# anonymous-author-918/deq-mpc-corl

Measured on AMD Instinct MI355X. Metric: QP solves/sec at (B,T=20,nx=13,nu=4), higher is better.
Workload: dtype f32

## Files before the change

### deq-mpc-corl_amd/_lib.py

```python
from __future__ import annotations

import ctypes as C
import os

_HERE = os.path.dirname(os.path.abspath(__file__))
LIB_PATH = os.environ.get("MI_ALQP_LIB") or os.path.join(_HERE, "csrc", "libmi_alqp.so")

ABI_VERSION = 17


class AlqpDims(C.Structure):
    _fields_ = [("B", C.c_int), ("T", C.c_int), ("nx", C.c_int), ("nu", C.c_int)]


class AlqpParams(C.Structure):
    _fields_ = [("al_iter", C.c_int), ("max_newton", C.c_int), ("n_ls", C.c_int),
                ("flags", C.c_int), ("rho_scale", C.c_double), ("variant", C.c_int),
                ("skip_flag", C.c_void_p), ("exit_tol", C.c_double), ("newton_counts", C.c_void_p),
                ("exit_scratch", C.c_void_p), ("quad_stagger", C.c_int)]


class AlqpTrace(C.Structure):
    _fields_ = [("g", C.c_void_p), ("d", C.c_void_p), ("phi", C.c_void_p),
                ("phi_prev", C.c_void_p), ("k", C.c_void_p), ("accept", C.c_void_p)]


class AlqpObstacles(C.Structure):
    _fields_ = [("pos", C.c_void_p), ("radius", C.c_double), ("nobs", C.c_int), ("state_estimator", C.c_int)]


class AlqpBwdDyn(C.Structure):
    _fields_ = [("lam", C.c_void_p), ("sb_lam", C.c_long), ("dF", C.c_void_p), ("dc", C.c_void_p), ("dx0", C.c_void_p)]


class AlqpIpmParams(C.Structure):
    _fields_ = [("flags", C.c_int), ("max_iter", C.c_int), ("iter0", C.c_int), ("kkt_eps", C.c_double),
                ("variant", C.c_int)]


class AlqpRigidParams(C.Structure):
    _fields_ = [("mass", C.c_double), ("J", C.c_double * 9), ("Jinv", C.c_double * 9), ("g", C.c_double * 3),
                ("motor_dist", C.c_double), ("kf", C.c_double), ("bf", C.c_double), ("km", C.c_double),
                ("act_scale", C.c_double), ("u_hover", C.c_double), ("pend_L", C.c_double), ("ss", C.c_double * 12),
                ("bf_force", C.c_double)]


IPM_VARIANTS = {"auto": 0, "generic_lds": 1, "generic_ws": 2, "resident": 3}


ALQP_IPM_INIT, ALQP_IPM_RESID, ALQP_IPM_STEP, ALQP_IPM_LOOP, ALQP_IPM_FINAL = 1, 2, 4, 8, 16
ALQP_INIT_MERIT = 1
ALQP_DUAL_UPDATE = 2
ALQP_SAVE_FACTOR = 4
ALQP_WS_PRIMED = 8
ALQP_EXIT_IN_KERNEL = 16
ALQP_E_COOP = -4
VARIANT_AUTO, VARIANT_TEAM, VARIANT_QUAD = 0, 1, 2

ERRORS = {-1: "bad argument", -2: "unsupported (nx, nu), or horizon / batch beyond what the requested kernel can hold or address",
          -3: "kernel launch failed", -4: "grid too large for a cooperative launch"}

_P = C.c_void_p
_ROWS = (_P, _P, C.c_int, C.c_long, C.c_long, C.c_long, C.c_long)
_SIGS = {
    "alqp_solve_nonlin": (C.c_int, [C.POINTER(AlqpDims), C.POINTER(AlqpParams), C.c_int, C.c_double, _P, _P, _P, _P, _P,
                                    C.c_long, C.c_long, _P, _P, _P, _P, _P, _P, _P, _P, C.c_size_t, _P]),
    "alqp_solve_nonlin_rows": (C.c_int, [C.POINTER(AlqpDims), C.POINTER(AlqpParams), C.c_int, C.c_double, _P, _P, _P, _P, _P,
                                         C.c_long, C.c_long, _P, _P, C.c_long, C.c_long, *_ROWS, _P, _P, _P, _P, _P, _P, _P,
                                         _P, C.POINTER(AlqpTrace), _P, C.c_size_t, _P]),
    "alqp_dyn_pendulum1l": (C.c_int, [C.c_long, _P, _P, C.c_double, _P, _P, _P, _P]),
    "alqp_dyn_cartpole1l": (C.c_int, [C.c_long, _P, _P, C.c_double, _P, _P, _P, _P]),
    "alqp_dyn_cartpole1l_v2": (C.c_int, [C.c_long, _P, _P, C.c_double, _P, _P, _P, _P]),
    "alqp_dyn_cartpole2l": (C.c_int, [C.c_long, _P, _P, C.c_double, _P, _P, _P, _P]),
    "alqp_dyn_rexquadrotor": (C.c_int, [C.c_long, C.POINTER(AlqpRigidParams), _P, _P, C.c_double, _P, _P, _P]),
    "alqp_dyn_flyingcartpole": (C.c_int, [C.c_long, C.POINTER(AlqpRigidParams), _P, _P, C.c_double, _P, _P, _P]),
    "alqp_solve_lin": (C.c_int, [C.POINTER(AlqpDims), C.POINTER(AlqpParams), _P, _P, _P, _P, _P, _P, _P,
                                 C.c_long, C.c_long, _P, _P, _P, _P, _P, _P, _P, _P,
                                 C.POINTER(AlqpTrace), _P, C.c_size_t, _P]),
    "alqp_solve_lin_shared": (C.c_int, [C.POINTER(AlqpDims), C.POINTER(AlqpParams), _P, _P, _P, _P,
                                        C.c_long, C.c_long, C.c_long, C.c_long, _P, _P, _P,
                                        C.c_long, C.c_long, _P, _P, _P, _P, _P, _P, _P, _P,
                                        C.POINTER(AlqpTrace), _P, C.c_size_t, _P]),
    "alqp_solve_lin_dense": (C.c_int, [C.POINTER(AlqpDims), C.POINTER(AlqpParams), _P, _P, _P, _P, _P, _P, _P,
                                       C.c_long, C.c_long, _P, _P, _P, _P, _P, _P, _P, _P,
                                       C.POINTER(AlqpTrace), _P]),
    "alqp_solve_lin_xbox": (C.c_int, [C.POINTER(AlqpDims), C.POINTER(AlqpParams), _P, _P, _P, _P, _P, _P, _P,
                                      C.c_long, C.c_long, _P, _P, C.c_long, C.c_long, _P, _P, _P, _P, _P, _P, _P, _P,
                                      C.POINTER(AlqpTrace), _P]),
    "alqp_solve_lin_poly": (C.c_int, [C.POINTER(AlqpDims), C.POINTER(AlqpParams), _P, _P, _P, _P, _P, _P, _P,
                                      C.c_long, C.c_long, _P, _P, C.c_int, C.c_long, C.c_long, C.c_long, C.c_long,
                                      _P, _P, _P, _P, _P, _P, _P, _P, C.POINTER(AlqpTrace), _P]),
    "alqp_solve_lin_gen": (C.c_int, [C.POINTER(AlqpDims), C.POINTER(AlqpParams), _P, _P, _P, _P, _P, _P, _P,
                                     C.c_long, C.c_long, _P, _P, _P, _P, _P, _P, _P, _P,
                                     C.POINTER(AlqpTrace), _P, C.c_size_t, _P,
                                     _P, _P, _P, C.c_long, C.c_long, _P, _P, C.c_int, C.c_long, C.c_long, C.c_long, C.c_long]),
    "alqp_newton_step": (C.c_int, [C.POINTER(AlqpDims), _P, _P, _P, _P, _P, _P, _P, _P, _P, _P,
                                   C.c_long, C.c_long, C.POINTER(AlqpObstacles), _P, C.c_size_t, _P, _P, _P, _P, _P]),
    "alqp_merit": (C.c_int, [C.POINTER(AlqpDims), C.c_int, _P, _P, _P, _P, _P, _P, _P, _P, _P,
                             C.c_long, C.c_long, C.POINTER(AlqpObstacles), _P, _P, _P]),
    "alqp_linesearch_pick": (C.c_int, [C.POINTER(AlqpDims), C.c_int, _P, _P, _P, _P, _P, _P, _P]),
    "alqp_dual_update": (C.c_int, [C.POINTER(AlqpDims), _P, _P, _P, _P, _P, C.c_long, C.c_long,
                                   C.POINTER(AlqpObstacles), _P, _P, C.c_double, _P]),
    "alqp_backward": (C.c_int, [C.POINTER(AlqpDims), _P, _P, C.c_size_t, _P, _P, _P, _P, _P, _P,
                                C.POINTER(AlqpBwdDyn), _P]),
    "alqp_merit_pick": (C.c_int, [C.POINTER(AlqpDims), C.c_int, _P, _P, _P, _P, _P, _P, _P, _P, _P,
                                  C.c_long, C.c_long, C.POINTER(AlqpObstacles), _P, _P, _P, _P, _P, _P, _P]),
    "alqp_newton_step_xbox": (C.c_int, [C.POINTER(AlqpDims), _P, _P, _P, _P, _P, _P, _P, _P, _P, _P,
                                        C.c_long, C.c_long, _P, _P, C.c_long, C.c_long, _P, _P, _P, _P, _P]),
# ... 75 lines not shown
```

### deq-mpc-corl_amd/csrc/alqp_quad.hip

```cpp
#if defined(ALQP_BWD_DYN_UNIT) || defined(ALQP_SHDYN_UNIT)
#undef ALQP_PHASE_TIMING
#endif
#include <hip/hip_runtime.h>

#include "alqp_quad.hpp"
#include "alqp_dims.hpp"
#include "alqp_launch.hpp"

#if defined(ALQP_QUAD_F32) == defined(ALQP_QUAD_F64)
#error "compile alqp_quad.hip with exactly one of -DALQP_QUAD_F32, -DALQP_QUAD_F64"
#endif

namespace alqp {

#ifndef ALQP_FUSE_LS
#define ALQP_FUSE_LS 1
#endif
#ifdef ALQP_PHASE_TIMING
__device__ unsigned long long g_phase_cycles[10];
#define QSTAMP(b) qd.stamp(b)
#else
#define QSTAMP(b)
#endif
#ifdef ALQP_SHDYN_UNIT
template <typename real, int NX, int NU, bool TRACE, class Dyn = NoDyn>
__global__ __launch_bounds__(64) __attribute__((amdgpu_waves_per_eu(1, 1))) void k_solve_lin_quad_shdyn(ShdynSolveArgs<real> a, TraceArgs<real> tr, real *ws) {
#else
template <typename real, int NX, int NU, bool TRACE, class Dyn = NoDyn>
__global__ __launch_bounds__(64) __attribute__((amdgpu_waves_per_eu(1, 1))) void k_solve_lin_quad(SolveArgs<real> a, TraceArgs<real> tr, real *ws) {
#endif
    using C = QCfg<real, NX, NU>;
    constexpr bool NL = Dyn::ID != 0;
#ifndef ALQP_FUSE_LS_F64
#define ALQP_FUSE_LS_F64 1
#endif
    constexpr bool FUSE_LS = ALQP_FUSE_LS && (sizeof(real) == 4 || ALQP_FUSE_LS_F64) && !NL;
    constexpr int N = C::N;
    if (a.skip && *a.skip != 0.0) return;
    const int lane = threadIdx.x, qi = lane >> 2;
    const int b_raw = blockIdx.x * 16 + qi;
    const bool active = b_raw < a.B;
    {
        int stag = a.stagger;
        const int mode = (a.flags >> 20) & 0xf;
        if ((a.flags >> 24) & 0xff) stag = (a.flags >> 24) & 0xff;
        if (stag > 0) {
            const unsigned hw = __builtin_amdgcn_s_getreg(4 | (0 << 6) | (31 << 11));
            int simd = (hw >> 4) & 3;
            if (mode == 1) simd = simd * 16 + ((hw >> 8) & 0xf);
            if (mode == 2) simd &= 1;
            if (mode == 3) simd = blockIdx.x & 1;
            if (mode == 4) simd = (simd & 1) ^ (blockIdx.x & 1);
            if (mode == 5) simd = (hw >> 8) & 3;
            for (int i = 0; i < simd * stag; ++i) __builtin_amdgcn_s_sleep(16);
        }
    }
#ifdef ALQP_ALIAS_ALL
    const int b = (active ? b_raw : a.B - 1) % ALQP_ALIAS_ALL;
#else
    const int b = active ? b_raw : a.B - 1;
#endif
    const int T = a.T, M = C::M(T);

    Quad<real, NX, NU> qd;
    __shared__ real w_lds[QCfg<real, NX, NU>::WLDS_WORDS];
    qd.wl = w_lds + threadIdx.x;
    qd.q = lane & 3;
    qd.T = T;
    qd.active = active;
    qd.gQd = a.Qd + (size_t)b * T * N;
    qd.gq = a.q + (size_t)b * T * N;
#ifdef ALQP_SHDYN_UNIT
    qd.gF = a.F + (size_t)b * a.sb_F;
    qd.gc = a.c + (size_t)b * a.sb_c;
    qd.mt_F = a.mt_F; qd.mt_c = a.mt_c;
#else
    qd.gF = a.F + (size_t)b * (T - 1) * NX * N;
    qd.gc = a.c + (size_t)b * (T - 1) * NX;
#endif
    qd.gx0 = a.x0 + (size_t)b * NX;
    qd.gulo = a.ulo + (size_t)b * a.sb_u;
    qd.guhi = a.uhi + (size_t)b * a.sb_u;
    qd.st_u = a.st_u;
    qd.gz = a.z + (size_t)b * T * N;
    qd.glam = a.lam + (size_t)b * M;
    qd.rec = ws + C::rec_base(b, T);
    qd.gFw = const_cast<real *>(qd.gF);
    qd.dyn_h = a.dyn_h;
    qd.rho = a.rho[b];
    qd.info = 0;
    real phi_prev = a.phi[b];
#ifdef ALQP_PHASE_TIMING
    for (int i = 0; i < 10; ++i) qd.tacc[i] = 0;
#endif
    QSTAMP(-1);
    if (!(a.flags & ALQP_WS_PRIMED)) {
        if constexpr (NL) qd.stage_in(false, false);
        else qd.stage_in(a.max_newton == 0 || a.al_iter == 0 || (a.flags & ALQP_EXIT_IN_KERNEL) ||
                         (!C::PHI0_FWD && (a.flags & ALQP_INIT_MERIT)));
    }
    const bool ref_exit = (a.flags & ALQP_EXIT_IN_KERNEL) != 0;
    int gphase = 0;

    int step_id = 0;
    bool pend = false;
    real alpha_pend = 0;
    int bad = 0;
    real rn2 = 0, phi_next = 0;
    for (int it = 0; it < a.al_iter; ++it) {
        bool phi_from_forward = false;
        if (a.flags & ALQP_INIT_MERIT) {
            if (it > 0) {
                phi_prev = phi_next;
            } else if (C::PHI0_FWD && a.max_newton > 0 && !ref_exit) {
                phi_from_forward = true;
            } else {
                if constexpr (NL) qd.template linearize<Dyn>(real(0), false);
                real p1[1];
                qd.template merit_candidates<1>(p1, true);
                phi_prev = p1[0];
            }
        }
        pend = false;
        double nrm_old = 0;
        int n_done = 0;
        if (ref_exit) {
            int bad0 = 0;
            const real r0 = it == 0 ? qd.rplus2(bad0) : rn2;
            nrm_old = sqrt(grid_sum_ordered(wave_sum_leaders(exit_term(r0, qor(qd.info)), active && qd.q == 0), a.exit_scratch, gphase));
        }
        for (int st = 0; st < a.max_newton; ++st, ++step_id) {
            real *tg = nullptr;
            if constexpr (TRACE) tg = (tr.g && active) ? tr.g + ((size_t)step_id * a.B + b) * T * N : nullptr;
            QSTAMP(9);
            if constexpr (NL) {
                qd.template linearize<Dyn>(alpha_pend, pend);
                pend = false;
            }
            qd.forward(tg, alpha_pend, pend, (phi_from_forward && st == 0) ? &phi_prev : nullptr);
            real ph[20];
            const bool store_s = !FUSE_LS || ref_exit || st + 1 == a.max_newton;
            qd.template backward<FUSE_LS>(ph, nullptr, store_s);
            QSTAMP(-1);
            if constexpr (TRACE) {
                if (tr.d && active) {
                    real *td = tr.d + ((size_t)step_id * a.B + b) * T * N;
                    for (int t = 0; t < T; ++t)
                        for (int j = qd.q; j < N; j += 4) td[t * N + j] = qd.recp(t)[C::wn(C::oY, j)];
                }
            }
            if constexpr (NL) qd.template merit_nonlin<Dyn>(ph);
            else if constexpr (!FUSE_LS) qd.template merit_candidates<20>(ph, false);
            QSTAMP(6);
            int kbest = 0;
            real best = ph[0];
#pragma unroll
            for (int k = 1; k < 20; ++k) {
                if (k < a.n_ls && !(best != best) && (ph[k] != ph[k] || ph[k] < best)) {
                    best = ph[k];
                    kbest = k;
                }
            }
            const bool acc = best < phi_prev;
            if constexpr (TRACE) {
                if (active && qd.q == 0) {
                    if (tr.phi)
#pragma unroll
                        for (int k = 0; k < 20; ++k)
                            if (k < a.n_ls) tr.phi[((size_t)step_id * a.n_ls + k) * a.B + b] = ph[k];
                    if (tr.phi_prev) tr.phi_prev[(size_t)step_id * a.B + b] = phi_prev;
                    if (tr.k) tr.k[(size_t)step_id * a.B + b] = kbest;
                    if (tr.accept) tr.accept[(size_t)step_id * a.B + b] = acc ? 1 : 0;
                }
            }
            const real alpha = acc ? real(1) / real(1 << kbest) : real(0);
            pend = true;
            alpha_pend = alpha;
            QSTAMP(7);
            phi_prev = best;
            if (ref_exit) {
                int bad1 = 0;
                real ph_unused = 0, r1 = 0;
                qd.template iter_end<Dyn>(alpha_pend, pend, false, (real)a.rho_scale, false, ph_unused, r1, bad1);
                pend = false;
                const double nw = sqrt(grid_sum_ordered(wave_sum_leaders(exit_term(r1, qor(qd.info)), active && qd.q == 0), a.exit_scratch, gphase));
                ++n_done;
                if (nw < a.exit_tol || fabs(nrm_old - nw) / nw < a.exit_tol) break;
                nrm_old = nw;
            }
        }
        if (ref_exit && a.newton_counts && blockIdx.x == 0 && lane == 0) a.newton_counts[it] = grid_barrier_timed_out(a.exit_scratch) ? -1 : n_done;
        bad = 0;
        qd.template iter_end<Dyn>(alpha_pend, pend, (a.flags & ALQP_DUAL_UPDATE) != 0, (real)a.rho_scale, it + 1 == a.al_iter,
                    phi_next, rn2, bad);
        pend = false;
// ... 231 lines not shown
```

### deq-mpc-corl_amd/csrc/alqp_quad.hpp

```cpp
#pragma once
#include <hip/hip_runtime.h>

#include <type_traits>

#include "alqp_team.hpp"
#include "alqp_dyn.hpp"

namespace alqp {

template <int Q>
__device__ inline float qb(float v) {
    return __builtin_bit_cast(float, __builtin_amdgcn_mov_dpp(__builtin_bit_cast(int, v), Q * 0x55, 0xF, 0xF, true));
}
template <int Q>
__device__ inline double qb(double v) {
    long long b = __builtin_bit_cast(long long, v);
    int lo = __builtin_amdgcn_mov_dpp((int)(b & 0xffffffffll), Q * 0x55, 0xF, 0xF, true);
    int hi = __builtin_amdgcn_mov_dpp((int)(b >> 32), Q * 0x55, 0xF, 0xF, true);
    return __builtin_bit_cast(double, ((long long)hi << 32) | (unsigned int)lo);
}
template <typename real>
__device__ inline real qbv(real v, int src) {
    switch (src & 3) {
        case 0: return qb<0>(v);
        case 1: return qb<1>(v);
        case 2: return qb<2>(v);
        default: return qb<3>(v);
    }
}
template <int CTRL>
__device__ inline float qperm(float v) {
    return __builtin_bit_cast(float, __builtin_amdgcn_mov_dpp(__builtin_bit_cast(int, v), CTRL, 0xF, 0xF, true));
}
template <int CTRL>
__device__ inline double qperm(double v) {
    long long b = __builtin_bit_cast(long long, v);
    int lo = __builtin_amdgcn_mov_dpp((int)(b & 0xffffffffll), CTRL, 0xF, 0xF, true);
    int hi = __builtin_amdgcn_mov_dpp((int)(b >> 32), CTRL, 0xF, 0xF, true);
    return __builtin_bit_cast(double, ((long long)hi << 32) | (unsigned int)lo);
}
template <typename real>
__device__ inline real qsum(real v) {
    v += qperm<0xB1>(v);
    v += qperm<0x4E>(v);
    return v;
}
__device__ inline int qor(int v) {
    v |= __builtin_amdgcn_mov_dpp(v, 0xB1, 0xF, 0xF, true);
    v |= __builtin_amdgcn_mov_dpp(v, 0x4E, 0xF, 0xF, true);
    return v;
}
template <typename real>
__device__ inline real sel4(real a0, real a1, real a2, real a3, int q) {
    real lo = (q & 1) ? a1 : a0, hi = (q & 1) ? a3 : a2;
    return (q & 2) ? hi : lo;
}

struct __attribute__((packed, aligned(4))) f4u { float x, y, z, w; };
struct __attribute__((packed, aligned(8))) d4u { double x, y, z, w; };
__device__ inline void gld4(const float *p, float &a, float &b, float &c, float &d) {
    f4u t = *reinterpret_cast<const f4u *>(p);
    a = t.x; b = t.y; c = t.z; d = t.w;
}
__device__ inline void gld4(const double *p, double &a, double &b, double &c, double &d) {
    d4u t = *reinterpret_cast<const d4u *>(p);
    a = t.x; b = t.y; c = t.z; d = t.w;
}
__device__ inline void gst4(float *p, float a, float b, float c, float d) {
    f4u t; t.x = a; t.y = b; t.z = c; t.w = d;
    *reinterpret_cast<f4u *>(p) = t;
}
__device__ inline void gst4(double *p, double a, double b, double c, double d) {
    d4u t; t.x = a; t.y = b; t.z = c; t.w = d;
    *reinterpret_cast<d4u *>(p) = t;
}
template <int LEN, typename real>
__device__ inline void gload(const real *p, real (&dst)[LEN]) {
#pragma unroll
    for (int c = 0; c + 4 <= LEN; c += 4) gld4(p + c, dst[c], dst[c + 1], dst[c + 2], dst[c + 3]);
#pragma unroll
    for (int c = (LEN / 4) * 4; c < LEN; ++c) dst[c] = p[c];
}

#ifndef ALQP_W_LDS
#define ALQP_W_LDS 1
#endif
#ifndef ALQP_EXP_NOQ
#define ALQP_EXP_NOQ 0
#endif
#ifndef ALQP_EXP_NORS
#define ALQP_EXP_NORS 0
#endif
#ifndef ALQP_EXP_NOL
#define ALQP_EXP_NOL 0
#endif
template <typename real, int SW, int N, bool IN_LDS>
struct WPanel {
    real a[SW][N];
    __device__ __forceinline__ real (&operator[](int s))[N] { return a[s]; }
    __device__ __forceinline__ const real (&operator[](int s) const)[N] { return a[s]; }
};
template <typename real, int N>
struct WRowLds {
    real *p;
    __device__ __forceinline__ real &operator[](int k) const { return p[k * 64]; }
};
template <typename real, int SW, int N>
struct WPanel<real, SW, N, true> {
    real *base;
    __device__ __forceinline__ WRowLds<real, N> operator[](int s) const { return WRowLds<real, N>{base + s * N * 64}; }
};
template <int LEN, typename real>
__device__ __forceinline__ void gload(const real *p, WRowLds<real, LEN> row) {
    real tmp[LEN];
    gload<LEN>(p, tmp);
#pragma unroll
    for (int k = 0; k < LEN; ++k) row[k] = tmp[k];
}

struct NoDyn {
    static constexpr int ID = 0;
};

struct Fld {
    int h, t;
};
template <int H, int T>
struct FldT {
    static constexpr int h = H, t = T;
    __host__ __device__ constexpr operator Fld() const { return {H, T}; }
};
template <typename real>
struct FRef {
    real *p;
    Fld f;
};
template <typename real, int H, int T>
__device__ __forceinline__ FRef<std::remove_const_t<real>> operator+(real *p, FldT<H, T>) {
    return {const_cast<std::remove_const_t<real> *>(p), Fld{H, T}};
}

template <typename real, int NX_, int NU_>
struct QCfg {
    static constexpr int NX = NX_, NU = NU_, N = NX_ + NU_;
    static constexpr int SH = (N + 3) / 4;
    static constexpr int SW = (NX + 3) / 4;
    static constexpr int SY = SH;
    static constexpr int HT = 2 * SH * (SH + 1);
    __host__ __device__ static constexpr int hidx(int s, int j) { return 2 * s * (s + 1) + j; }
    static constexpr int ST = 2 * SW * (SW + 1);
    static constexpr int BLK = 64 / (int)sizeof(real);
#ifndef ALQP_REC_IL_F32
#define ALQP_REC_IL_F32 2
#endif
    static constexpr int IL = sizeof(real) == 4 ? ALQP_REC_IL_F32 : 1;
    static_assert(IL == 1 || BLK == 16, "groups of 16 words are 64-byte blocks");
    __host__ __device__ static constexpr int w(int x) { return (x / 16) * (16 * IL) + x % 16; }
    static constexpr int NLAST = N - 4 * (SH - 1);
    __host__ __device__ static constexpr int lanes_of(int s) { return s == SH - 1 ? NLAST : 4; }
    __host__ __device__ static constexpr int lstride(int s) { return lanes_of(s) == 3 ? 16 : 4 * lanes_of(s); }
    __host__ __device__ static constexpr int lbase(int s) {
        int o = 0;
        for (int i = 0; i < s; ++i) o += (i + 1) * lstride(i);
        return o;
    }
    static constexpr int LW = lbase(SH);
    static constexpr bool PHI0_FWD = sizeof(real) == 4;
#ifndef ALQP_S_AFTER_F32
#define ALQP_S_AFTER_F32 0
#endif
    static constexpr bool S_AFTER = sizeof(real) == 8 || ALQP_S_AFTER_F32;
#ifndef ALQP_W_LDS_F32
#define ALQP_W_LDS_F32 0
#endif
    static constexpr bool W_LDS = ALQP_W_LDS && (sizeof(real) == 8 || ALQP_W_LDS_F32);
    static constexpr int WLDS_WORDS = W_LDS ? SW * N * 64 : 1;
    __host__ __device__ static constexpr int p4(int x) { return (x + 3) & ~3; }
    static constexpr int NF = 9;
    __host__ __device__ static constexpr int fslots(int i) { return (i <= 1 || i == 6 || i == 7) ? SY : (i == 5 ? 4 : SW); }
    static constexpr int oL = 2 * 16 * (SY / 4);
    __host__ __device__ static constexpr int tail_at(int i) {
        int g = (oL + LW + 15) & ~15, o = 0;
        for (int k = 0; k < NF; ++k) {
            const int r = fslots(k) % 4;
            if (r > 0 && o + r > 4) { g += 16; o = 0; }
            if (k == i) return g + o;
            o += r;
        }
        return o > 0 ? g + 16 : g;
    }
    __host__ __device__ static constexpr int head_at(int i) {
        if (i < 2) return i * 16 * (SY / 4);
        int o = tail_at(NF);
        for (int k = 2; k < i; ++k) o += 16 * (fslots(k) / 4);
        return o;
    }
    static constexpr FldT<head_at(0), tail_at(0)> oY{};
    static constexpr FldT<head_at(1), tail_at(1)> oZ{};
    static constexpr FldT<head_at(2), tail_at(2)> oR{};
    static constexpr FldT<head_at(3), tail_at(3)> oS{};
    static constexpr FldT<head_at(4), tail_at(4)> oLE{};
    static_assert(NU <= 4, "the u-slot layout holds one control per lane");
    static constexpr FldT<head_at(5), tail_at(5)> oUS{};
    static constexpr FldT<head_at(6), tail_at(6)> oQ{};
    static constexpr FldT<head_at(7), tail_at(7)> oq{};
    static constexpr FldT<head_at(8), tail_at(8)> oC{};
    static constexpr int RECW = (head_at(NF) + 31) & ~31;
    static_assert(IL == 1 || RECW % 16 == 0, "whole groups per record");
    template <int S>
    __host__ __device__ static constexpr int lp(int m, int q) {
        return m < 4 * (S / 4) ? 16 * (m / 4) + 4 * q + m % 4 : 16 * (S / 4) + q * (S % 4) + m - 4 * (S / 4);
    }
    template <int S>
    __host__ __device__ static constexpr int fw(Fld f, int p) {
        return p < 16 * (S / 4) ? w(f.h + p) : w(f.t + 4 * ((p - 16 * (S / 4)) / (S % 4)) + (p - 16 * (S / 4)) % (S % 4));
    }
    __host__ __device__ static constexpr int pn(int k) { return lp<SY>(k >> 2, k & 3); }
    __host__ __device__ static constexpr int px(int r) { return lp<SW>(r >> 2, r & 3); }
    __host__ __device__ static constexpr int wn(Fld f, int k) { return fw<SY>(f, pn(k)); }
    __host__ __device__ static constexpr int M(int T) { return T * NX + 2 * T * NU; }
    static constexpr int RSTR = RECW * IL;
    __host__ __device__ static constexpr size_t rec_base(int b, int T) { return (size_t)(b / IL) * T * RSTR + (size_t)(b % IL) * 16; }
    __host__ __device__ static constexpr size_t ws_words(int B, int T) { return (size_t)((B + IL - 1) / IL) * T * RSTR; }
    __host__ static bool ws_covers(int B, int T) {
        return rec_base(B - 1, T) + (size_t)(T - 1) * RSTR + w(RECW - 1) + 1 <= ws_words(B, T);
    }
};

template <typename real, int NX, int NU>
struct Quad {
    using C = QCfg<real, NX, NU>;
    static constexpr int N = C::N, SH = C::SH, SW = C::SW, SY = C::SY, HT = C::HT, ST = C::ST, RECW = C::RECW;

    int q, T;
    bool active;
    const real *gQd, *gq, *gF, *gc, *gx0, *gulo, *guhi;
    long st_u;
#ifdef ALQP_SHDYN_UNIT
    int mt_F, mt_c;
#endif
    real *gz, *glam, *rec;
    real rho;
    int info;
    real *wl;
    using WT = WPanel<real, SW, N, C::W_LDS>;
    __device__ __forceinline__ WT wpanel() const {
        if constexpr (C::W_LDS) return WT{wl};
        else return WT{};
    }
    real *gFw;
    real dyn_h;
    const real *gobs;
    int nobs;
    real obs_r2;
    bool no_init;

    __device__ __forceinline__ real uhi(int t, int j) const { return guhi[t * st_u + j]; }
    __device__ __forceinline__ real ulo(int t, int j) const { return gulo[t * st_u + j]; }
    __device__ __forceinline__ real *recp(int t) const { return rec + (size_t)t * C::RSTR; }
#ifdef ALQP_PHASE_TIMING
    unsigned long long tacc[10], tlast;
    __device__ __forceinline__ void stamp(int bucket) {
        unsigned long long now;
        __builtin_amdgcn_sched_barrier(0);
        asm volatile("s_waitcnt vmcnt(0)\n\ts_memtime %0\n\ts_waitcnt lgkmcnt(0)" : "=s"(now)::"memory");
        __builtin_amdgcn_sched_barrier(0);
        if (bucket >= 0) tacc[bucket] += now - tlast;
        tlast = now;
    }
#define ALQP_STAMP(b) stamp(b)
#else
#define ALQP_STAMP(b)
#endif

    template <int S, int L>
    __device__ __forceinline__ void ld_slots(FRef<real> f, real (&v)[L]) const {
        static_assert(L <= S, "slots of the field");
#pragma unroll
        for (int c = 0; 4 * c < L && c < S / 4; ++c) {
            const real *p = f.p + C::w(f.f.h + 16 * c) + 4 * q;
            if (4 * c + 3 < L) gld4(p, v[4 * c], v[4 * c + 1], v[4 * c + 2], v[4 * c + 3]);
            else
#pragma unroll
                for (int i = 0; 4 * c + i < L; ++i) v[4 * c + i] = p[i];
        }
        constexpr int H = 4 * (S / 4), R = S % 4;
        if constexpr (L > H) {
            const real *p = f.p + C::w(f.f.t) + 4 * q;
#pragma unroll
            for (int m = H; m < L; ++m) v[m] = p[m - H];
        }
    }
    template <int S, int L0>
    __device__ __forceinline__ void ld_slots_from(FRef<real> f, real (&v)[S]) const {
        static_assert(L0 >= 0 && L0 <= S, "slots of the field");
#pragma unroll
        for (int c = L0 / 4; c < S / 4; ++c) {
            const real *p = f.p + C::w(f.f.h + 16 * c) + 4 * q;
            if (4 * c >= L0) gld4(p, v[4 * c], v[4 * c + 1], v[4 * c + 2], v[4 * c + 3]);
            else {
                real w[4];
                gld4(p, w[0], w[1], w[2], w[3]);
#pragma unroll
                for (int i = 0; i < 4; ++i)
                    if (4 * c + i >= L0) v[4 * c + i] = w[i];
            }
        }
        constexpr int H = 4 * (S / 4);
// ... 285 lines not shown
        const real a0 = sel4(real(1), real(0.5), real(0.25), real(0.125), q);
        for (int t = 0; t < T; ++t) {
            const bool dyn = t < T - 1;
            const real *rp = recp(t), *rn = recp(dyn ? t + 1 : t);
            real zt[N], dt[N], Qt[N], qt[N], zn[NX], dn[NX], le[NX], lu[NU], ll[NU], bu[NU], bl[NU];
            ld_rep_n(rp + C::oZ, zt);
            ld_rep_n(rp + C::oY, dt);
            ld_rep_n(rp + C::oQ, Qt);
            ld_rep_n(rp + C::oq, qt);
            ld_repx_of_n(rn + C::oZ, zn);
            ld_repx_of_n(rn + C::oY, dn);
            ld_rep_x(rp + C::oLE, le);
            ld_rep_us(rp, lu, ll, bu, bl);
            real alpha = a0;
#pragma unroll
            for (int i = 0; i < 5; ++i) {
                real zc[N];
                real acc = 0;
#pragma unroll
                for (int j = 0; j < N; ++j) {
                    zc[j] = fma_(alpha, dt[j], zt[j]);
                    acc = fma_(fma_(real(0.5) * Qt[j], zc[j], qt[j]), zc[j], acc);
                }
#pragma unroll
                for (int ju = 0; ju < NU; ++ju) {
                    const real vu = zc[NX + ju] - bu[ju], vl = bl[ju] - zc[NX + ju];
                    const real cu = fmax_(vu, real(0)), cl = fmax_(vl, real(0));
                    acc += fma_(lu[ju], vu, ll[ju] * vl) + real(0.5) * rho * fma_(cu, cu, cl * cl);
                }
                if (dyn) {
                    real xn[NX];
                    dyn_value<Dyn, real>(zc, dyn_h, xn);
#pragma unroll
                    for (int r = 0; r < NX; ++r) {
                        const real rr = fma_(alpha, dn[r], zn[r]) - xn[r];
                        acc = fma_(fma_(real(0.5) * rho, rr, le[r]), rr, acc);
                    }
                }
                if (t == 0) {
#pragma unroll
                    for (int r = 0; r < NX; ++r) {
                        const real rr = zc[r] - x0v[r];
                        acc = fma_(fma_(real(0.5) * rho, rr, li[r]), rr, acc);
                    }
                }
                m[i] += acc;
                alpha *= real(0.0625);
            }
        }
#pragma unroll
        for (int k = 0; k < 20; ++k) phi[k] = qbv(m[k >> 2], k);
    }

    template <bool EXT = false>
    __device__ __forceinline__ void forward(real *g_out, real alpha, bool pending, real *phi0, const real *gxn = nullptr) {
        real mdist = 0;
        real S[ST], Sy[SW];
        real vpo[SW], Syo[SW];
        real zc[SW];
#pragma unroll
        for (int i = 0; i < ST; ++i) S[i] = 0;
#pragma unroll
        for (int s = 0; s < SW; ++s) Sy[s] = 0;
        {
            real z0[SW], xi[SW], li[SW], r0[SW];
            if constexpr (EXT) {
                ld_own_ext<NX>(gz, z0);
                ld_own_ext<NX>(glam + (T - 1) * NX, li);
            } else {
                ld_ownx_of_n(recp(0) + C::oZ, z0);
                ld_own_x(recp(T - 1) + C::oLE, li);
            }
            ld_own_ext<NX>(gx0, xi);
            if (pending) {
                real d0[SW];
                ld_ownx_of_n(recp(0) + C::oY, d0);
#pragma unroll
                for (int s = 0; s < SW; ++s) z0[s] = fma_(alpha, d0[s], z0[s]);
            }
#pragma unroll
            for (int s = 0; s < SW; ++s) {
                bool valid = 4 * s + 3 < NX || 4 * s + q < NX;
                if constexpr (EXT) valid = valid && !no_init;
                const real r = valid ? z0[s] - xi[s] : real(0);
                vpo[s] = valid ? fma_(rho, r, li[s]) : real(0);
                if constexpr (C::PHI0_FWD) mdist += valid ? fma_(fma_(real(0.5) * rho, r, li[s]), r, real(0)) : real(0);
                Syo[s] = 0;
                r0[s] = r;
                zc[s] = z0[s];
            }
            if (!EXT && active) st_own_x(recp(T - 1) + C::oR, r0);
        }
        for (int t = 0; t < T; ++t) {
            const bool dyn = t < T - 1;
            WT W = wpanel();
            real Y[N];
            real dio[SY];
            real v[SW];
            real zs[SY];
            real hob[3] = {0, 0, 0};
            real *rp = recp(t);
            {
                real zt[N];
                real Qo[SY], qo[SY];
                real cs[SW], zn[SW], lm[SW];
                real lu, ll, bu, bl;
                const int td = dyn ? t : (T > 1 ? T - 2 : 0);
// ... 197 lines not shown
                    constexpr int KB = 8;
                    real wj[SW];
#pragma unroll
                    for (int s = 0; s < SW; ++s) wj[s] = W[s][j];
#pragma unroll
                    for (int k0 = j + 1; k0 < N; k0 += KB) {
                        real wv[KB][SW];
#pragma unroll
                        for (int kk = 0; kk < KB; ++kk)
#pragma unroll
                            for (int s = 0; s < SW; ++s)
                                if (k0 + kk < N) wv[kk][s] = W[s][k0 + kk];
                        __builtin_amdgcn_sched_barrier(0);
#pragma unroll
                        for (int kk = 0; kk < KB; ++kk) {
                            const int k = k0 + kk;
                            if (k < N) {
                                const real lkj = qbv(H[C::hidx(k >> 2, j)], k) * ip;
#pragma unroll
                                for (int s = (k >> 2); s < SH; ++s) H[C::hidx(s, k)] = fma_(-H[C::hidx(s, j)], lkj, H[C::hidx(s, k)]);
#pragma unroll
                                for (int s = 0; s < SW; ++s) W[s][k] = fma_(-wj[s], lkj, wv[kk][s]);
                                Y[k] = fma_(-Y[j], lkj, Y[k]);
                            }
                        }
                    }
                } else {
#pragma unroll
                for (int k = j + 1; k < N; ++k) {
                    const real lkj = qbv(H[C::hidx(k >> 2, j)], k) * ip;
#pragma unroll
                    for (int s = (k >> 2); s < SH; ++s) H[C::hidx(s, k)] = fma_(-H[C::hidx(s, j)], lkj, H[C::hidx(s, k)]);
#pragma unroll
                    for (int s = 0; s < SW; ++s) W[s][k] = fma_(-W[s][j], lkj, W[s][k]);
                    Y[k] = fma_(-Y[j], lkj, Y[k]);
                }
                }
                if constexpr (C::S_AFTER) ipv[j] = ip;
                if (!C::S_AFTER && dyn) {
#pragma unroll
                    for (int b = 0; b < NX; ++b) {
                        const real wbj = qbv(W[b >> 2][j], b) * ip;
#pragma unroll
                        for (int s = (b >> 2); s < SW; ++s) S[C::hidx(s, b)] = fma_(W[s][j], wbj, S[C::hidx(s, b)]);
                    }
                    const real yip = Y[j] * ip;
#pragma unroll
                    for (int s = 0; s < SW; ++s) Sy[s] = fma_(W[s][j], yip, Sy[s]);
                }
                H[C::hidx(j >> 2, j)] = (q == (j & 3)) ? ip : H[C::hidx(j >> 2, j)];
            }
            ALQP_STAMP(2);
            if (active) {
                if (!(ALQP_EXP_NOL && t >= T - ALQP_EXP_NOL))
#pragma unroll
                for (int s = 0; s < SH; ++s)
#pragma unroll
                    for (int c = 0; c <= s; ++c)
                        if (C::lanes_of(s) == 4 || q < C::lanes_of(s))
                            gst4(lchunk(rp, s, c, q), H[C::hidx(s, 4 * c)],
                                 H[C::hidx(s, 4 * c + 1)], H[C::hidx(s, 4 * c + 2)], H[C::hidx(s, 4 * c + 3)]);
                real yo[SY];
                own_of<N, SY>(Y, yo);
                st_own_n(rp + C::oY, yo);
                if (pending) st_own_n(rp + C::oZ, zs);
            }

            if constexpr (C::S_AFTER) {
                if (dyn) {
#pragma unroll
                    for (int j = 0; j < N; ++j) {
#pragma unroll
                        for (int b = 0; b < NX; ++b) {
                            const real wbj = qbv(W[b >> 2][j], b) * ipv[j];
#pragma unroll
                            for (int s = (b >> 2); s < SW; ++s) S[C::hidx(s, b)] = fma_(W[s][j], wbj, S[C::hidx(s, b)]);
                        }
                        const real yip = Y[j] * ipv[j];
#pragma unroll
                        for (int s = 0; s < SW; ++s) Sy[s] = fma_(W[s][j], yip, Sy[s]);
                    }
                }
            }
#pragma unroll
            for (int s = 0; s < SW; ++s) {
                vpo[s] = v[s];
                Syo[s] = Sy[s];
            }
            ALQP_STAMP(3);
        }
        if constexpr (C::PHI0_FWD) { if (phi0) *phi0 = qsum(mdist); }
    }

    __host__ __device__ static constexpr int lane_lo(int m, int j) { return m == (j >> 2) ? (j & 3) + 1 : 0; }
    __device__ __forceinline__ bool in_lanes(int lo, int hi) const {
        return lo == 0 ? q < hi : (hi == 4 ? q >= lo : (q >= lo && q < hi));
    }
    __device__ __forceinline__ void lsolve_own(const real (&H)[HT], real (&u)[SY]) const {
#pragma unroll
        for (int j = 0; j < N; ++j) {
            const int mj = j >> 2;
            const real wj = qbv(u[mj] * H[C::hidx(mj, j)], j);
#pragma unroll
            for (int m = mj; m < SH; ++m) {
                const int lo = lane_lo(m, j);
                if (lo >= C::lanes_of(m)) continue;
                const real v = fma_(-H[C::hidx(m, j)], wj, u[m]);
                u[m] = lo == 0 ? v : (q >= lo ? v : u[m]);
            }
        }
    }
    __device__ __forceinline__ void ltsolve_own(const real (&H)[HT], const real (&y)[SY], real (&d)[SY], real (&rep)[N]) const {
#pragma unroll
        for (int m = 0; m < SY; ++m) d[m] = 0;
#pragma unroll
        for (int i = N - 1; i >= 0; --i) {
            const int mi = i >> 2;
            real p = 0;
            bool any = false;
#pragma unroll
            for (int m = mi; m < SH; ++m) {
                const int lo = lane_lo(m, i), hi = C::lanes_of(m);
                if (lo >= hi) continue;
                const real h = (lo == 0 && hi == 4) ? H[C::hidx(m, i)] : (in_lanes(lo, hi) ? H[C::hidx(m, i)] : real(0));
                p = any ? fma_(h, d[m], p) : h * d[m];
                any = true;
            }
            real r = y[mi];
            if (any) r -= qsum(p);
            const real di = qbv(r * H[C::hidx(mi, i)], i);
            rep[i] = di;
            d[mi] = (q == (i & 3)) ? di : d[mi];
        }
    }

    template <bool LS>
    __device__ __forceinline__ void backward(real (&phi)[20], real *d_ext = nullptr, bool store_s = true) {
        constexpr int MU0 = NX / 4;
        real c0 = 0, c1 = 0, c2 = 0;
        real acc[20];
        real rvT[SW], lvT[SW];
#pragma unroll
        for (int k = 0; k < 20; ++k) acc[k] = 0;
#pragma unroll
        for (int s = 0; s < SW; ++s) rvT[s] = lvT[s] = 0;
        real dxs[SW];
#pragma unroll
        for (int s = 0; s < SW; ++s) dxs[s] = 0;
        for (int t = T - 1; t >= 0; --t) {
            const bool dyn = t < T - 1;
            real *rp = recp(t);
            real H[HT];
            if (ALQP_EXP_NOL && t >= T - ALQP_EXP_NOL) {
#pragma unroll
                for (int i = 0; i < HT; ++i) H[i] = real(1);
            } else
#pragma unroll
            for (int s = 0; s < SH; ++s)
#pragma unroll
                for (int c = 0; c <= s; ++c) {
                    const int ql = (C::lanes_of(s) == 4 || q < C::lanes_of(s)) ? q : 0;
                    gld4(lchunk(rp, s, c, ql), H[C::hidx(s, 4 * c)],
                         H[C::hidx(s, 4 * c + 1)], H[C::hidx(s, 4 * c + 2)], H[C::hidx(s, 4 * c + 3)]);
                }
            real yo[SY];
            ld_own_n(rp + C::oY, yo);
            WT W = wpanel();
            load_F_rows(dyn ? t : (T > 1 ? T - 2 : 0), W);
            real zz[SY], QQ[SY], qq[SY], rv[SW], lv[SW];
            real lu = 0, ll = 0, bu = 0, bl = 0;
            if constexpr (LS) {
                ld_own_n(rp + C::oZ, zz);
                if constexpr (ALQP_EXP_NOQ) { for (int m = 0; m < SY; ++m) QQ[m] = real(1); }
                else ld_own_n(rp + C::oQ, QQ);
                ld_own_n(rp + C::oq, qq);
                ld_own_us(rp, lu, ll, bu, bl);
                if constexpr (ALQP_EXP_NORS) { for (int s = 0; s < SW; ++s) rv[s] = real(0); }
                else ld_own_x(rp + C::oR, rv);
                ld_own_x(rp + C::oLE, lv);
            }
            ALQP_STAMP(4);
            if (dyn) {
                real vv[N];
#pragma unroll
                for (int j = 0; j < N; ++j) {
                    real p = 0;
#pragma unroll
                    for (int s = 0; s < SW; ++s) p = fma_(W[s][j], dxs[s], p);
                    vv[j] = qsum(p);
                }
                real uo[SY];
                own_of<N, SY>(vv, uo);
                lsolve_own(H, uo);
#pragma unroll
                for (int m = 0; m < SY; ++m) yo[m] = fma_(rho, uo[m], yo[m]);
            }
            real down[SY], Y[N];
            ltsolve_own(H, yo, down, Y);
            if (active) {
                if (d_ext) st_own_ext<N>(d_ext + t * N, down);
                else st_own_n(rp + C::oY, down);
            }
            real sv[SW];
#pragma unroll
            for (int s = 0; s < SW; ++s) sv[s] = 0;
// ... 348 lines not shown
```

### include/mi_alqp.h

```cpp
#ifndef MI_ALQP_H
#define MI_ALQP_H

#include <stddef.h>

#ifdef __cplusplus
extern "C" {
#endif

typedef struct AlqpDims {
    int B;
    int T;
    int nx;
    int nu;
} AlqpDims;

typedef struct AlqpObstacles {
    const void *pos;
    double radius;
    int nobs;
    int state_estimator;
} AlqpObstacles;

#define ALQP_INIT_MERIT   1
#define ALQP_DUAL_UPDATE  2
#define ALQP_SAVE_FACTOR  4
#define ALQP_WS_PRIMED    8

#define ALQP_EXIT_IN_KERNEL 16

typedef struct AlqpParams {
    int al_iter;
    int max_newton;
    int n_ls;
    int flags;
    double rho_scale;
    int variant;
    const double *skip_flag;
    double exit_tol;
    int *newton_counts;
    double *exit_scratch;
    int quad_stagger;
} AlqpParams;

typedef struct AlqpTrace {
    void *g;
    void *d;
    void *phi;
    void *phi_prev;
    int *k;
    int *accept;
} AlqpTrace;

#define ALQP_E_BADARG     (-1)
#define ALQP_E_UNSUPPORTED (-2)
#define ALQP_E_LAUNCH     (-3)
#define ALQP_E_COOP       (-4)

int alqp_supported(const AlqpDims *dims, int is_f64);
int alqp_supported_variant(const AlqpDims *dims, int is_f64, int variant);
int alqp_pick_variant(const AlqpDims *dims, int is_f64, int flags, long quad_min_batch);
size_t alqp_lds_bytes(const AlqpDims *dims, int is_f64);
int alqp_qps_per_wave(const AlqpDims *dims, int is_f64);
size_t alqp_workspace_bytes(const AlqpDims *dims, int is_f64);

int alqp_solve_lin_f32(const AlqpDims *dims, const AlqpParams *prm, const void *Qd, const void *q,
                       const void *F, const void *c, const void *x0, const void *u_lo,
                       const void *u_hi, long sb_u, long st_u, void *z, void *lam, void *rho,
                       void *phi, void *rnorm2, int *info, unsigned char *status,
                       void *factor_out, const AlqpTrace *trace, void *workspace, size_t ws_bytes,
                       void *stream);
int alqp_solve_lin_f64(const AlqpDims *dims, const AlqpParams *prm, const void *Qd, const void *q,
                       const void *F, const void *c, const void *x0, const void *u_lo,
                       const void *u_hi, long sb_u, long st_u, void *z, void *lam, void *rho,
                       void *phi, void *rnorm2, int *info, unsigned char *status,
                       void *factor_out, const AlqpTrace *trace, void *workspace, size_t ws_bytes,
                       void *stream);

int alqp_solve_lin_shared_f32(const AlqpDims *dims, const AlqpParams *prm, const void *Qd, const void *q,
                              const void *F, const void *c, long sb_F, long st_F, long sb_c, long st_c,
                              const void *x0, const void *u_lo, const void *u_hi, long sb_u, long st_u, void *z,
                              void *lam, void *rho, void *phi, void *rnorm2, int *info, unsigned char *status,
// ... 334 lines not shown
```

Measured before the change: 6.252 million.

## Keep first KL stages of Riccati factor in LDS instead of workspace

For f32 quad kernels where W is not in LDS, the per-stage Cholesky factor written in the forward pass and read back in the backward pass is kept in shared memory for the first KL time steps. Global workspace stores happen only for the remaining stages, or when the factor must persist for the final or ref-exit iteration. This cuts global-memory round trips between forward and backward. In exchange it uses up to about 36KB of LDS per block, which may limit occupancy, and adds a flag and extra branching.

```diff
diff --git a/deq-mpc-corl_amd/_lib.py b/deq-mpc-corl_amd/_lib.py
--- a/deq-mpc-corl_amd/_lib.py
+++ b/deq-mpc-corl_amd/_lib.py
@@ -54,6 +54,7 @@
 ALQP_SAVE_FACTOR = 4
 ALQP_WS_PRIMED = 8
 ALQP_EXIT_IN_KERNEL = 16
+ALQP_FACTOR_IN_WS = 32
 ALQP_E_COOP = -4
 VARIANT_AUTO, VARIANT_TEAM, VARIANT_QUAD = 0, 1, 2
 
diff --git a/deq-mpc-corl_amd/csrc/alqp_quad.hip b/deq-mpc-corl_amd/csrc/alqp_quad.hip
--- a/deq-mpc-corl_amd/csrc/alqp_quad.hip
+++ b/deq-mpc-corl_amd/csrc/alqp_quad.hip
@@ -65,6 +65,12 @@
     Quad<real, NX, NU> qd;
     __shared__ real w_lds[QCfg<real, NX, NU>::WLDS_WORDS];
     qd.wl = w_lds + threadIdx.x;
+    constexpr bool FL = C::KL > 0;
+    if constexpr (FL) {
+        __shared__ __attribute__((aligned(16))) real l_lds[C::KL * C::FLW];
+        qd.fl = (ALQP_LDS real *)l_lds;
+        qd.kl = (a.flags & ALQP_FACTOR_IN_WS) ? 0 : (T < C::KL ? T : C::KL);
+    }
     qd.q = lane & 3;
     qd.T = T;
     qd.active = active;
@@ -137,10 +143,11 @@
                 qd.template linearize<Dyn>(alpha_pend, pend);
                 pend = false;
             }
-            qd.forward(tg, alpha_pend, pend, (phi_from_forward && st == 0) ? &phi_prev : nullptr);
+            if constexpr (FL) qd.fl_ws = ref_exit || (it + 1 == a.al_iter && st + 1 == a.max_newton);
+            qd.template forward<false, FL>(tg, alpha_pend, pend, (phi_from_forward && st == 0) ? &phi_prev : nullptr);
             real ph[20];
             const bool store_s = !FUSE_LS || ref_exit || st + 1 == a.max_newton;
-            qd.template backward<FUSE_LS>(ph, nullptr, store_s);
+            qd.template backward<FUSE_LS, FL>(ph, nullptr, store_s);
             QSTAMP(-1);
             if constexpr (TRACE) {
                 if (tr.d && active) {
diff --git a/deq-mpc-corl_amd/csrc/alqp_quad.hpp b/deq-mpc-corl_amd/csrc/alqp_quad.hpp
--- a/deq-mpc-corl_amd/csrc/alqp_quad.hpp
+++ b/deq-mpc-corl_amd/csrc/alqp_quad.hpp
@@ -73,6 +73,19 @@
 __device__ inline void gst4(double *p, double a, double b, double c, double d) {
     d4u t; t.x = a; t.y = b; t.z = c; t.w = d;
     *reinterpret_cast<d4u *>(p) = t;
+}
+#define ALQP_LDS __attribute__((address_space(3)))
+template <typename real>
+__device__ inline void lld4(const ALQP_LDS real *p, real &a, real &b, real &c, real &d) {
+    typedef real v4 __attribute__((ext_vector_type(4)));
+    const v4 t = *(const ALQP_LDS v4 *)p;
+    a = t.x; b = t.y; c = t.z; d = t.w;
+}
+template <typename real>
+__device__ inline void lst4(ALQP_LDS real *p, real a, real b, real c, real d) {
+    typedef real v4 __attribute__((ext_vector_type(4)));
+    v4 t; t.x = a; t.y = b; t.z = c; t.w = d;
+    *(ALQP_LDS v4 *)p = t;
 }
 template <int LEN, typename real>
 __device__ inline void gload(const real *p, real (&dst)[LEN]) {
@@ -175,6 +188,22 @@
 #endif
     static constexpr bool W_LDS = ALQP_W_LDS && (sizeof(real) == 8 || ALQP_W_LDS_F32);
     static constexpr int WLDS_WORDS = W_LDS ? SW * N * 64 : 1;
+    __host__ __device__ static constexpr int fl_chunk(int s) { return 16 * 4 * lanes_of(s); }
+    __host__ __device__ static constexpr int fl_base(int s) {
+        int o = 0;
+        for (int i = 0; i < s; ++i) o += (i + 1) * fl_chunk(i);
+        return o;
+    }
+    static constexpr int FLW = fl_base(SH);
+    static constexpr int FL_BUDGET = 36 * 1024 / 4;
+#ifndef ALQP_FACTOR_LDS_F32
+#define ALQP_FACTOR_LDS_F32 -1
+#endif
+    static constexpr int KL = (sizeof(real) != 4 || W_LDS) ? 0
+                              : ALQP_FACTOR_LDS_F32 >= 0   ? ALQP_FACTOR_LDS_F32
+                              : N > 17                     ? 0
+                              : (FL_BUDGET / FLW < 8 ? FL_BUDGET / FLW : 8);
+    static_assert(KL * FLW <= 40 * 1024 / 4, "four wavefronts' factor stages fit a CU's LDS");
     __host__ __device__ static constexpr int p4(int x) { return (x + 3) & ~3; }
     static constexpr int NF = 9;
     __host__ __device__ static constexpr int fslots(int i) { return (i <= 1 || i == 6 || i == 7) ? SY : (i == 5 ? 4 : SW); }
@@ -254,6 +283,60 @@
     int nobs;
     real obs_r2;
     bool no_init;
+    ALQP_LDS real *fl;
+    int kl;
+    bool fl_ws;
+    __device__ __forceinline__ void fstage(int t, ALQP_LDS real *&pl, ALQP_LDS real *&pc) const {
+        int lane;
+        asm volatile("v_mbcnt_lo_u32_b32 %0, -1, 0\n\tv_mbcnt_hi_u32_b32 %0, -1, %0" : "=v"(lane));
+        pl = fl + t * C::FLW + 4 * lane;
+        pc = fl + t * C::FLW + 4 * C::NLAST * (lane >> 2);
+    }
+    __device__ __forceinline__ ALQP_LDS real *fchunk(ALQP_LDS real *pl, ALQP_LDS real *pc, int s, int c, int ql) const {
+        return (C::lanes_of(s) == 4 ? pl : pc + 4 * ql) + C::fl_base(s) + c * C::fl_chunk(s);
+    }
+    __device__ __forceinline__ void st_factor_ws(real *rp, const real (&H)[HT]) const {
+#pragma unroll
+        for (int s = 0; s < SH; ++s)
+#pragma unroll
+            for (int c = 0; c <= s; ++c)
+                if (C::lanes_of(s) == 4 || q < C::lanes_of(s))
+                    gst4(lchunk(rp, s, c, q), H[C::hidx(s, 4 * c)],
+                         H[C::hidx(s, 4 * c + 1)], H[C::hidx(s, 4 * c + 2)], H[C::hidx(s, 4 * c + 3)]);
+    }
+    __device__ __forceinline__ void st_factor_lds(int t, const real (&H)[HT]) const {
+        ALQP_LDS real *pl, *pc;
+        fstage(t, pl, pc);
+#pragma unroll
+        for (int s = 0; s < SH; ++s)
+#pragma unroll
+            for (int c = 0; c <= s; ++c)
+                if (C::lanes_of(s) == 4 || q < C::lanes_of(s))
+                    lst4<real>(fchunk(pl, pc, s, c, q), H[C::hidx(s, 4 * c)],
+                         H[C::hidx(s, 4 * c + 1)], H[C::hidx(s, 4 * c + 2)], H[C::hidx(s, 4 * c + 3)]);
+    }
+    __device__ __forceinline__ void ld_factor_ws(real *rp, real (&H)[HT]) const {
+#pragma unroll
+        for (int s = 0; s < SH; ++s)
+#pragma unroll
+            for (int c = 0; c <= s; ++c) {
+                const int ql = (C::lanes_of(s) == 4 || q < C::lanes_of(s)) ? q : 0;
+                gld4(lchunk(rp, s, c, ql), H[C::hidx(s, 4 * c)],
+                     H[C::hidx(s, 4 * c + 1)], H[C::hidx(s, 4 * c + 2)], H[C::hidx(s, 4 * c + 3)]);
+            }
+    }
+    __device__ __forceinline__ void ld_factor_lds(int t, real (&H)[HT]) const {
+        ALQP_LDS real *pl, *pc;
+        fstage(t, pl, pc);
+#pragma unroll
+        for (int s = 0; s < SH; ++s)
+#pragma unroll
+            for (int c = 0; c <= s; ++c) {
+                const int ql = (C::lanes_of(s) == 4 || q < C::lanes_of(s)) ? q : 0;
+                lld4<real>(fchunk(pl, pc, s, c, ql), H[C::hidx(s, 4 * c)],
+                     H[C::hidx(s, 4 * c + 1)], H[C::hidx(s, 4 * c + 2)], H[C::hidx(s, 4 * c + 3)]);
+            }
+    }
 
     __device__ __forceinline__ real uhi(int t, int j) const { return guhi[t * st_u + j]; }
     __device__ __forceinline__ real ulo(int t, int j) const { return gulo[t * st_u + j]; }
@@ -645,7 +728,7 @@
         for (int k = 0; k < 20; ++k) phi[k] = qbv(m[k >> 2], k);
     }
 
-    template <bool EXT = false>
+    template <bool EXT = false, bool FL = false>
     __device__ __forceinline__ void forward(real *g_out, real alpha, bool pending, real *phi0, const real *gxn = nullptr) {
         real mdist = 0;
         real S[ST], Sy[SW];
@@ -949,6 +1032,9 @@
             }
             ALQP_STAMP(2);
             if (active) {
+                if constexpr (FL) {
+                    if (t >= kl || fl_ws) st_factor_ws(rp, H);
+                } else
                 if (!(ALQP_EXP_NOL && t >= T - ALQP_EXP_NOL))
 #pragma unroll
                 for (int s = 0; s < SH; ++s)
@@ -962,6 +1048,9 @@
                 st_own_n(rp + C::oY, yo);
                 if (pending) st_own_n(rp + C::oZ, zs);
             }
+            if constexpr (FL) {
+                if (t < kl) st_factor_lds(t, H);
+            }
 
             if constexpr (C::S_AFTER) {
                 if (dyn) {
@@ -1031,7 +1120,7 @@
         }
     }
 
-    template <bool LS>
+    template <bool LS, bool FL = false>
     __device__ __forceinline__ void backward(real (&phi)[20], real *d_ext = nullptr, bool store_s = true) {
         constexpr int MU0 = NX / 4;
         real c0 = 0, c1 = 0, c2 = 0;
@@ -1048,6 +1137,11 @@
             const bool dyn = t < T - 1;
             real *rp = recp(t);
             real H[HT];
+            if constexpr (FL) {
+                static_assert(!FL || !ALQP_EXP_NOL, "the no-factor experiment runs with the factor in the records");
+                if (t < kl) ld_factor_lds(t, H);
+                else ld_factor_ws(rp, H);
+            } else
             if (ALQP_EXP_NOL && t >= T - ALQP_EXP_NOL) {
 #pragma unroll
                 for (int i = 0; i < HT; ++i) H[i] = real(1);
diff --git a/include/mi_alqp.h b/include/mi_alqp.h
--- a/include/mi_alqp.h
+++ b/include/mi_alqp.h
@@ -27,6 +27,7 @@
 #define ALQP_WS_PRIMED    8
 
 #define ALQP_EXIT_IN_KERNEL 16
+#define ALQP_FACTOR_IN_WS 32
 
 typedef struct AlqpParams {
     int al_iter;
```

Result: faster. 6.553 million, median of 6 (+4.8%).
